# MSNLAB/Federated-Lifelong-Person-ReID

Hardware: AMD Instinct MI355X
Metric: images/sec (whole node) per fed round, fedstil resnet50 (higher is better)
Workload: dtype bf16; 1 GPU; model=resnet50-fedstil, global_batch=64, img=128x64, images_per_round_per_client=512, num_classes=8000, lambda_k=2000, rehearsal_set=2000 exemplar budget + task (m=32/id), parallelism=fed-dp1 (1 client/GPU)

## Files before the change

flreid_amd/models/resnet.py:

```python

from __future__ import annotations

from typing import List, Type, Union

import torch
import torch.nn as nn
import torch.nn.functional as F

from flreid_amd import ops
from flreid_amd.tools.logger import Logger
from flreid_amd.tools.winit import weights_init_classifier, weights_init_kaiming

_log = Logger("models.resnet")


class EvalFusedBatchNorm2d(nn.BatchNorm2d):

    fuse_relu = False

    def forward(self, x):
        if not self.training:
            out = ops.bn_eval_2d(x, self, relu=self.fuse_relu)
            if out is not None:
                return out
        else:
            out = ops.bn_train_2d(x, self, relu=self.fuse_relu)
            if out is not None:
                return out
        out = super().forward(x)
        return F.relu(out, inplace=True) if self.fuse_relu else out


class EvalFusedBatchNorm1d(nn.BatchNorm1d):

    def forward(self, x):
        if not self.training:
            out = ops.bn_eval_2d(x, self)
            if out is not None:
                return out
        else:
            out = ops.bn_train_2d(x, self)
            if out is not None:
                return out
        return super().forward(x)


class FusedConv3x3(nn.Conv2d):

    def forward(self, x):
        if self.stride == (1, 1) and self.bias is None:
            y = ops.conv3x3_try(x, self.weight)
            if y is not None:
                return y
        return super().forward(x)


def conv3x3(cin: int, cout: int, stride: int = 1) -> nn.Conv2d:
    return FusedConv3x3(cin, cout, 3, stride=stride, padding=1, bias=False)


def conv1x1(cin: int, cout: int, stride: int = 1) -> nn.Conv2d:
    return nn.Conv2d(cin, cout, 1, stride=stride, bias=False)


class BasicBlock(nn.Module):
    expansion = 1

    def __init__(self, cin: int, planes: int, stride: int = 1,
                 downsample: nn.Module = None):
        super().__init__()
        self.conv1 = conv3x3(cin, planes, stride)
        self.bn1 = EvalFusedBatchNorm2d(planes)
        self.bn1.fuse_relu = True
        self.relu = nn.ReLU(inplace=True)
        self.conv2 = conv3x3(planes, planes)
        self.bn2 = EvalFusedBatchNorm2d(planes)
        self.downsample = downsample

    def forward(self, x: torch.Tensor) -> torch.Tensor:
        identity = x if self.downsample is None else self.downsample(x)
        out = self.bn1(self.conv1(x))
        out = self.bn2(self.conv2(out))
        return self.relu(out + identity)


class Bottleneck(nn.Module):
    expansion = 4

    def __init__(self, cin: int, planes: int, stride: int = 1,
                 downsample: nn.Module = None):
        super().__init__()
        self.conv1 = conv1x1(cin, planes)
        self.bn1 = EvalFusedBatchNorm2d(planes)
        self.bn1.fuse_relu = True
        self.conv2 = conv3x3(planes, planes, stride)
        self.bn2 = EvalFusedBatchNorm2d(planes)
        self.bn2.fuse_relu = True
        self.conv3 = conv1x1(planes, planes * self.expansion)
        self.bn3 = EvalFusedBatchNorm2d(planes * self.expansion)
        self.relu = nn.ReLU(inplace=True)
        self.downsample = downsample

    def forward(self, x: torch.Tensor) -> torch.Tensor:
        identity = x if self.downsample is None else self.downsample(x)
        out = self.bn1(self.conv1(x))
        out = self.bn2(self.conv2(out))
        out = self.bn3(self.conv3(out))
        return self.relu(out + identity)


class ResNetTrunk(nn.Module):

    def __init__(self, block: Type[Union[BasicBlock, Bottleneck]],
                 layers: List[int], last_stride: int = 2):
        super().__init__()
        self.inplanes = 64
        self.conv1 = nn.Conv2d(3, 64, 7, stride=2, padding=3, bias=False)
        self.bn1 = EvalFusedBatchNorm2d(64)
        self.bn1.fuse_relu = True
        self.relu = nn.ReLU(inplace=True)
        self.maxpool = nn.MaxPool2d(3, stride=2, padding=1)
        self.layer1 = self._make_stage(block, 64, layers[0])
        self.layer2 = self._make_stage(block, 128, layers[1], stride=2)
        self.layer3 = self._make_stage(block, 256, layers[2], stride=2)
        self.layer4 = self._make_stage(block, 512, layers[3], stride=last_stride)
        self.avgpool = nn.AdaptiveAvgPool2d(1)
        self._init_weights()

    def _make_stage(self, block, planes: int, depth: int, stride: int = 1) -> nn.Sequential:
        downsample = None
        if stride != 1 or self.inplanes != planes * block.expansion:
            downsample = nn.Sequential(
                conv1x1(self.inplanes, planes * block.expansion, stride),
                EvalFusedBatchNorm2d(planes * block.expansion),
            )
        blocks = [block(self.inplanes, planes, stride, downsample)]
        self.inplanes = planes * block.expansion
        blocks += [block(self.inplanes, planes) for _ in range(1, depth)]
        return nn.Sequential(*blocks)

    def _init_weights(self) -> None:
        for m in self.modules():
            if isinstance(m, nn.Conv2d):
                nn.init.kaiming_normal_(m.weight, mode="fan_out", nonlinearity="relu")
            elif isinstance(m, nn.BatchNorm2d):
                nn.init.constant_(m.weight, 1.0)
                nn.init.constant_(m.bias, 0.0)

    def forward(self, x: torch.Tensor) -> torch.Tensor:
        x = self.maxpool(self.bn1(self.conv1(x)))
        x = self.layer4(self.layer3(self.layer2(self.layer1(x))))
        x = self.avgpool(x)
        return torch.flatten(x, 1)


_ARCH = {
    "resnet18": (BasicBlock, [2, 2, 2, 2], 512),
    "resnet34": (BasicBlock, [3, 4, 6, 3], 512),
    "resnet50": (Bottleneck, [3, 4, 6, 3], 2048),
    "resnet101": (Bottleneck, [3, 4, 23, 3], 2048),
    "resnet152": (Bottleneck, [3, 8, 36, 3], 2048),
}


class ResNetReID(nn.Module):
    def __init__(self, model_name: str, num_classes: int = 1000,
                 last_stride: int = 2, neck: str = "no",
                 pretrained: bool = False, **kwargs):
        super().__init__()
        for n, p in kwargs.items():
            setattr(self, n, p)
        if model_name not in _ARCH:
            raise ValueError(f"No model named {model_name}.")
        block, layers, self.in_planes = _ARCH[model_name]
        self.model_name = model_name
        self.num_classes = num_classes
        self.neck = neck
        self.base = ResNetTrunk(block, layers, last_stride=last_stride)

        if neck == "no":
            self.classifier = nn.Linear(self.in_planes, num_classes)
        elif neck == "bnneck":
            self.bottleneck = EvalFusedBatchNorm1d(self.in_planes)
            self.bottleneck.bias.requires_grad_(False)
            self.classifier = nn.Linear(self.in_planes, num_classes, bias=False)
            self.bottleneck.apply(weights_init_kaiming)
            self.classifier.apply(weights_init_classifier)
        else:
            raise ValueError(f"Mismatched neck type {neck}.")

# ... 58 lines not shown
```

flreid_amd/ops/__init__.py:

```python

from __future__ import annotations

import os
from collections import OrderedDict
from typing import Dict, Optional, Sequence, Tuple

import torch

from flreid_amd.ops import reference as ref

_EXT = None
_EXT_ERR: Optional[str] = None

_F32, _BF16 = 0, 1


def _load_extension():
    global _EXT, _EXT_ERR
    if _EXT is not None or _EXT_ERR is not None:
        return _EXT
    try:
        from flreid_amd.ops import _flreid_hip

        _EXT = _flreid_hip
# ... 770 lines not shown

def _penalty_meta(rows, n_sets: int, total: int, chunk: int):
    ptr_rows = [(p.data_ptr(), *(0 if t is None else t.data_ptr()
                                 for t in slots)) for p, slots in rows]
    key = (n_sets, rows[0][0].device,
           tuple((p.numel(), *pr) for (p, _), pr in zip(rows, ptr_rows)))
    meta = _PENALTY_META.get(key)
    if meta is not None:
        _PENALTY_META.move_to_end(key)
        return meta
    chunk_rows, offsets, flat_off = _chunk_table(
        [p.numel() for p, _ in rows], chunk, pad_to=4)
    assert flat_off == total
    dev = rows[0][0].device
    meta = (torch.tensor(ptr_rows, dtype=torch.int64, device=dev),
            torch.tensor(chunk_rows, dtype=torch.int32, device=dev),
            n_sets, offsets, total)
    _PENALTY_META[key] = meta
    while len(_PENALTY_META) > _PENALTY_META_CAP:
        _PENALTY_META.popitem(last=False)
    return meta


class _QuadraticPenaltyHipFn(torch.autograd.Function):

    @staticmethod
    def forward(ctx, meta, consts, *params):
        ext = _ext_or_raise("penalty_fwd")
        ptrs, chunks, n_sets, offsets, total = meta
        partials = torch.empty(chunks.shape[0], device=params[0].device,
                               dtype=torch.float32)
        ext.penalty_fwd(ptrs.data_ptr(), chunks.data_ptr(), n_sets,
                        partials.data_ptr(), chunks.shape[0], _stream())
        ctx.save_for_backward(*params)
        ctx.meta = meta
        ctx.consts = consts
        return partials.sum()

    @staticmethod
    def backward(ctx, grad_out):
        ext = _ext_or_raise("penalty_bwd")
        params = ctx.saved_tensors
        ptrs, chunks, n_sets, offsets, total = ctx.meta
        g = grad_out.to(torch.float32).contiguous()
        flat = torch.empty(total, device=g.device, dtype=torch.float32)
        ext.penalty_bwd(ptrs.data_ptr(), chunks.data_ptr(), n_sets,
                        g.data_ptr(), flat.data_ptr(), chunks.shape[0],
                        _stream())
        views = [torch.as_strided(flat, p.shape, p.stride(), off)
                 for p, off in zip(params, offsets)]
        return (None, None, *views)


def quadratic_penalty_sets(
        params: Dict[str, torch.Tensor],
        sets: Sequence[Tuple[Dict[str, torch.Tensor],
                             Optional[Dict[str, torch.Tensor]]]],
) -> torch.Tensor:
    sets = list(sets)
    first = next(iter(params.values()), None)
    if (sets and first is not None and first.is_cuda
            and os.environ.get("FLREID_NO_FUSED_PENALTY", "0") != "1"):
        plan = _penalty_plan(params, sets)
        if plan is not None:
            ext = _ext_or_raise("penalty_fwd")
            if ext is not None:
                rows, total = plan
                meta = _penalty_meta(rows, len(sets), total,
                                     ext.penalty_chunk())
                consts = tuple(t for _, slots in rows for t in slots
                               if t is not None)
                return _QuadraticPenaltyHipFn.apply(
                    meta, consts, *(p for p, _ in rows))
    return ref.quadratic_penalty_sets(params, sets)


def quadratic_penalty(params: Dict[str, torch.Tensor],
                      anchors: Dict[str, torch.Tensor],
                      importance: Optional[Dict[str, torch.Tensor]] = None,
                      ) -> torch.Tensor:
    return quadratic_penalty_sets(params, [(anchors, importance)])


class _BnTrain2dFn(torch.autograd.Function):

    @staticmethod
    def forward(ctx, x, gamma, beta, running_mean, running_var, momentum, eps,
                nbt, relu):
        ext = _ext_or_raise("bn_train")
        c = x.shape[1]
        m = x.numel() // c
        y = torch.empty_like(x)
        smean = torch.empty(c, device=x.device, dtype=torch.float32)
        sinv = torch.empty(c, device=x.device, dtype=torch.float32)
        nslab = ext.bn_train_nslab(m, c)
        part = torch.empty(2, nslab, c, device=x.device, dtype=torch.float32)
        has_rs = running_mean is not None
        ext.bn_train_fwd(
            x.data_ptr(), y.data_ptr(),
            gamma.detach().contiguous().data_ptr(),
            beta.detach().contiguous().data_ptr(),
            running_mean.data_ptr() if has_rs else 0,
            running_var.data_ptr() if has_rs else 0,
            smean.data_ptr(), sinv.data_ptr(),
            part[0].data_ptr(), part[1].data_ptr(),
            nbt.data_ptr() if nbt is not None else 0, m, c,
            float(momentum), float(eps), float(m) / float(m - 1),
            int(relu), _dt(x), _stream())
        ctx.save_for_backward(x, gamma, beta, smean, sinv)
        ctx.relu = bool(relu)
        return y

    @staticmethod
    def backward(ctx, dy):
        x, gamma, beta, smean, sinv = ctx.saved_tensors
        if x.dim() == 4:
            if not dy.is_contiguous(memory_format=torch.channels_last):
                dy = dy.contiguous(memory_format=torch.channels_last)
        elif not dy.is_contiguous():
            dy = dy.contiguous()
        if dy.dtype != x.dtype:
            dy = dy.to(x.dtype)
        ext = _ext_or_raise("bn_train")
        c = x.shape[1]
        m = x.numel() // c
        dx = torch.empty_like(x)
        dgamma = torch.empty(c, device=x.device, dtype=torch.float32)
        dbeta = torch.empty(c, device=x.device, dtype=torch.float32)
        nslab = ext.bn_train_nslab(m, c)
        part = torch.empty(2, nslab, c, device=x.device, dtype=torch.float32)
        ext.bn_train_bwd(x.data_ptr(), dy.data_ptr(), dx.data_ptr(),
                         gamma.detach().contiguous().data_ptr(),
                         beta.detach().contiguous().data_ptr(),
                         smean.data_ptr(), sinv.data_ptr(),
                         dgamma.data_ptr(), dbeta.data_ptr(),
                         part[0].data_ptr(), part[1].data_ptr(),
                         m, c, int(ctx.relu), _dt(x), _stream())
        return dx, dgamma, dbeta, None, None, None, None, None, None


def bn_train_2d(x: torch.Tensor, bn,
                relu: bool = False) -> Optional[torch.Tensor]:
    if os.environ.get("FLREID_NO_FUSED_BN", "0") == "1":
        return None
    if (not x.is_cuda or x.dtype not in (torch.float32, torch.bfloat16)
            or bn.weight is None or bn.bias is None):
        return None
    if x.dim() == 4:
        if not x.is_contiguous(memory_format=torch.channels_last):
            return None
    elif x.dim() == 2:
        if not x.is_contiguous():
            return None
    else:
        return None
    c = x.shape[1]
    m = x.numel() // c
    if c % 64 != 0 or m < 2 or m > 16384:
        return None
    if bn.momentum is None:
        return None
    if not extension_available():
        return None
    nbt = None
    if bn.track_running_stats and bn.running_mean is not None:
        nbt = bn.num_batches_tracked
        rm, rv = bn.running_mean, bn.running_var
    else:
        rm = rv = None
    return _BnTrain2dFn.apply(x, bn.weight, bn.bias, rm, rv,
                              bn.momentum, bn.eps, nbt, relu)


def _cl(t: torch.Tensor) -> torch.Tensor:
    return t if t.is_contiguous(memory_format=torch.channels_last) \
        else t.contiguous(memory_format=torch.channels_last)


def compose_theta_bf16(ext, gw: torch.Tensor, atten: Optional[torch.Tensor],
                       aw: Optional[torch.Tensor],
                       out: Optional[torch.Tensor] = None) -> torch.Tensor:
    gw_d = gw.detach()
    L, inner = atten_geometry(gw_d)
    if atten is not None and atten.numel() != L:
        if gw_d.dim() == 4 or not atten.numel() or L % atten.numel():
            raise ValueError(f"compose_theta_bf16: {atten.numel()} atten "
                             f"entries do not fit a last weight dim of {L}")
        L = atten.numel()
    if out is None:
        out = torch.empty_like(gw_d, dtype=torch.bfloat16)
    elif out.dtype != torch.bfloat16 or not same_layout(out, gw_d):
        raise ValueError("compose_theta_bf16: out must be bf16 in gw's layout")
    ext.compose2(gw_d.data_ptr(),
                 atten.detach().float().contiguous().data_ptr() if atten is not None else 0,
                 aw.detach().data_ptr() if aw is not None else 0,
                 out.data_ptr(), gw_d.numel(), L, inner, _dt(gw_d), _BF16,
                 _stream())
    return out


class _AdaptiveLinear1x1Fn(torch.autograd.Function):

    @staticmethod
    def forward(ctx, x, gw2d, atten, aw2d, bias):
        ext = _ext_or_raise("compose2")
        x_bf = x.detach().to(torch.bfloat16).contiguous()
        theta = compose_theta_bf16(ext, gw2d, atten, aw2d)
        y = x_bf @ theta.t()
        if bias is not None:
            y = y + bias.detach().to(torch.bfloat16)
        ctx.save_for_backward(x_bf, theta)
        ctx.x_dtype = x.dtype
        ctx.has_bias = bias is not None
        return y

    @staticmethod
    def backward(ctx, grad_out):
        x_bf, theta = ctx.saved_tensors
        g = grad_out.to(torch.bfloat16)
        dx = (g @ theta).to(ctx.x_dtype)
        d_aw = (g.t() @ x_bf).to(torch.float32)
        d_bias = grad_out.sum(0).to(torch.float32) if ctx.has_bias else None
        return dx, None, None, d_aw, d_bias


class _ThetaLinearFn(torch.autograd.Function):

    @staticmethod
    def forward(ctx, x, theta, bias, k2):
        x_bf = x.detach().to(torch.bfloat16).contiguous()
        th = theta.detach()
        if k2:
            ext = _ext_or_raise("theta_linear_fwd")
            m, k = x_bf.shape
            n = th.shape[0]
            y = torch.empty(m, n, device=x.device, dtype=torch.bfloat16)
            ext.theta_linear_fwd(
                x_bf.data_ptr(), th.data_ptr(),
                bias.detach().contiguous().float().data_ptr()
                if bias is not None else 0,
                y.data_ptr(), m, n, k, _stream())
        else:
            y = x_bf @ th.t()
            if bias is not None:
                y = y + bias.detach().to(torch.bfloat16)
        ctx.save_for_backward(x_bf, th)
        ctx.x_dtype = x.dtype
        ctx.has_bias = bias is not None
        return y

    @staticmethod
    def backward(ctx, grad_out):
        x_bf, th = ctx.saved_tensors
        g = grad_out.to(torch.bfloat16)
# ... 311 lines not shown
```

flreid_amd/ops/csrc/bn_train.hip:

```cpp

#include "common.h"
#include "ops.h"

namespace flreid {

template <typename T>
__device__ __forceinline__ void bn_load4(const T* p, float v[4]);

template <>
__device__ __forceinline__ void bn_load4<float>(const float* p, float v[4]) {
  const float4 t = *reinterpret_cast<const float4*>(p);
  v[0] = t.x; v[1] = t.y; v[2] = t.z; v[3] = t.w;
}

template <>
__device__ __forceinline__ void bn_load4<__hip_bfloat16>(
    const __hip_bfloat16* p, float v[4]) {
  const ushort4 t = *reinterpret_cast<const ushort4*>(p);
  v[0] = __bfloat162float(*(const __hip_bfloat16*)&t.x);
  v[1] = __bfloat162float(*(const __hip_bfloat16*)&t.y);
  v[2] = __bfloat162float(*(const __hip_bfloat16*)&t.z);
  v[3] = __bfloat162float(*(const __hip_bfloat16*)&t.w);
}

template <typename T>
__device__ __forceinline__ void bn_store4(T* p, const float v[4]);

template <>
__device__ __forceinline__ void bn_store4<float>(float* p, const float v[4]) {
  *reinterpret_cast<float4*>(p) = float4{v[0], v[1], v[2], v[3]};
}

template <>
__device__ __forceinline__ void bn_store4<__hip_bfloat16>(
    __hip_bfloat16* p, const float v[4]) {
  ushort4 t;
  __hip_bfloat16 b;
  b = __float2bfloat16(v[0]); t.x = *(const unsigned short*)&b;
  b = __float2bfloat16(v[1]); t.y = *(const unsigned short*)&b;
  b = __float2bfloat16(v[2]); t.z = *(const unsigned short*)&b;
  b = __float2bfloat16(v[3]); t.w = *(const unsigned short*)&b;
  *reinterpret_cast<ushort4*>(p) = t;
}

constexpr int BN_STRIPES = 16;
constexpr int BN_CG = 64;

template <typename T, bool IS_BWD>
__global__ __launch_bounds__(256) void bn_partial_kernel(
    const T* __restrict__ X, const T* __restrict__ DY,
    const float* __restrict__ smean, const float* __restrict__ sinv,
    const float* __restrict__ gamma, const float* __restrict__ beta,
    float* __restrict__ part_a, float* __restrict__ part_b, int64_t M,
    int C, int relu) {
  const int c0 = blockIdx.x * BN_CG;
  const int q = threadIdx.x & 15;
  const int r = threadIdx.x >> 4;
  const int c = c0 + q * 4;
  const int S = gridDim.y * BN_STRIPES;
  const int g = blockIdx.y * BN_STRIPES + r;

  __shared__ float la[BN_STRIPES][BN_CG + 4];
  __shared__ float lb[BN_STRIPES][BN_CG + 4];

  float mn[4], iv[4], sc[4], sh[4];
  if (IS_BWD) {
#pragma unroll
    for (int j = 0; j < 4; ++j) {
      mn[j] = smean[c + j];
      iv[j] = sinv[c + j];
      if (relu) {
        sc[j] = gamma[c + j] * iv[j];
        sh[j] = beta[c + j] - mn[j] * sc[j];
      }
    }
  }

  float sa[4] = {0.f, 0.f, 0.f, 0.f};
  float sb[4] = {0.f, 0.f, 0.f, 0.f};
  for (int64_t row = g; row < M; row += S) {
    float x[4];
    bn_load4(X + row * C + c, x);
// ... 152 lines not shown
      float d = dy[j];
      if (relu && x[j] * g_iv[j] + sh[j] <= 0.f) d = 0.f;
      dx[j] = g_iv[j] * (d - mdy[j] - xhat * mdyx[j]);
    }
    bn_store4(DX + row * C + c, dx);
  }
}

static int bn_nslab(int64_t M, int C) {
  const int cg = C / BN_CG;
  int ns = 256 / cg;
  const int max_rows = (int)((M + BN_STRIPES - 1) / BN_STRIPES);
  if (ns > max_rows) ns = max_rows;
  if (ns > 64) ns = 64;
  if (ns < 1) ns = 1;
  return ns;
}

extern "C" int flreid_bn_train_nslab(int64_t M, int C) {
  return bn_nslab(M, C);
}

extern "C" void flreid_bn_train_fwd(const void* X, void* Y, const float* gamma,
                                    const float* beta, float* rmean,
                                    float* rvar, float* smean, float* sinv,
                                    float* part_a, float* part_b,
                                    unsigned long long* nbt, int64_t M, int C,
                                    float momentum, float eps, float unbiased,
                                    int relu, int dtype, hipStream_t stream) {
  if (C % BN_CG != 0) throw std::runtime_error("bn_train: C % 64 != 0");
  dim3 grid(C / BN_CG, bn_nslab(M, C)), block(256);
  if (dtype == kBF16) {
    hipLaunchKernelGGL((bn_partial_kernel<__hip_bfloat16, false>), grid,
                       block, 0, stream, (const __hip_bfloat16*)X, nullptr,
                       nullptr, nullptr, nullptr, nullptr, part_a, part_b, M,
                       C, 0);
    hipLaunchKernelGGL(bn_finalize_fwd_kernel<__hip_bfloat16>, grid, block, 0,
                       stream, (const __hip_bfloat16*)X, (__hip_bfloat16*)Y,
                       gamma, beta, rmean, rvar, smean, sinv, part_a, part_b,
                       nbt, M, C, momentum, eps, unbiased, relu);
  } else {
    hipLaunchKernelGGL((bn_partial_kernel<float, false>), grid, block, 0,
                       stream, (const float*)X, nullptr, nullptr, nullptr,
                       nullptr, nullptr, part_a, part_b, M, C, 0);
    hipLaunchKernelGGL(bn_finalize_fwd_kernel<float>, grid, block, 0, stream,
                       (const float*)X, (float*)Y, gamma, beta, rmean, rvar,
                       smean, sinv, part_a, part_b, nbt, M, C, momentum, eps,
                       unbiased, relu);
  }
  HIP_CHECK(hipGetLastError());
}

extern "C" void flreid_bn_train_bwd(const void* X, const void* DY, void* DX,
                                    const float* gamma, const float* beta,
                                    const float* smean, const float* sinv,
                                    float* dgamma, float* dbeta,
                                    float* part_a, float* part_b, int64_t M,
                                    int C, int relu, int dtype,
                                    hipStream_t stream) {
  if (C % BN_CG != 0) throw std::runtime_error("bn_train: C % 64 != 0");
  dim3 grid(C / BN_CG, bn_nslab(M, C)), block(256);
  if (dtype == kBF16) {
    hipLaunchKernelGGL((bn_partial_kernel<__hip_bfloat16, true>), grid, block,
                       0, stream, (const __hip_bfloat16*)X,
                       (const __hip_bfloat16*)DY, smean, sinv, gamma, beta,
                       part_a, part_b, M, C, relu);
    hipLaunchKernelGGL(bn_finalize_bwd_kernel<__hip_bfloat16>, grid, block, 0,
                       stream, (const __hip_bfloat16*)X,
                       (const __hip_bfloat16*)DY, (__hip_bfloat16*)DX, gamma,
                       beta, smean, sinv, dgamma, dbeta, part_a, part_b, M, C,
                       relu);
  } else {
    hipLaunchKernelGGL((bn_partial_kernel<float, true>), grid, block, 0,
                       stream, (const float*)X, (const float*)DY, smean, sinv,
                       gamma, beta, part_a, part_b, M, C, relu);
    hipLaunchKernelGGL(bn_finalize_bwd_kernel<float>, grid, block, 0, stream,
                       (const float*)X, (const float*)DY, (float*)DX, gamma,
                       beta, smean, sinv, dgamma, dbeta, part_a, part_b, M, C,
                       relu);
  }
  HIP_CHECK(hipGetLastError());
}

}
```

flreid_amd/ops/csrc/module.cpp:

```cpp

#include <pybind11/pybind11.h>
#include <pybind11/stl.h>

#include <cstdint>
#include <stdexcept>
#include <string>
#include <vector>

#include "ops.h"

namespace py = pybind11;
using namespace flreid;

template <typename T> struct py_arg {
  using type = T;
  static T to(T v) { return v; }
};
template <typename T> struct py_arg<T*> {
  using type = uintptr_t;
  static T* to(uintptr_t v) { return reinterpret_cast<T*>(v); }
};
template <auto Fn> struct binder;
template <typename R, typename... A, R (*Fn)(A...)> struct binder<Fn> {
  static R call(typename py_arg<A>::type... a) {
    return Fn(py_arg<A>::to(a)...);
  }
};

#define FLREID_DEF(name) m.def(#name, &binder<&flreid_##name>::call)

PYBIND11_MODULE(_flreid_hip, m) {
  m.doc() = "flreid MI355X (gfx950) kernels";

  FLREID_DEF(l2norm_rows);
  FLREID_DEF(ce_smooth);
  FLREID_DEF(compose);
  FLREID_DEF(compose2);
  FLREID_DEF(bn_eval);
  FLREID_DEF(pairwise);
  FLREID_DEF(rowsq);
  FLREID_DEF(window_attn_fwd);
  FLREID_DEF(window_attn_bwd);
  FLREID_DEF(triplet_fwd);
  FLREID_DEF(triplet_bwd);
  FLREID_DEF(adaptive_linear_fwd);
  FLREID_DEF(theta_linear_fwd);
  FLREID_DEF(conv3x3_fwd);
  FLREID_DEF(conv3x3_tile);
  FLREID_DEF(conv3x3_img_fwd);
  FLREID_DEF(conv3x3_img_fwd_ldsw);
  FLREID_DEF(conv3x3_wgrad);
  FLREID_DEF(transpose_bf16);
  FLREID_DEF(bn_train_nslab);
  FLREID_DEF(bn_train_fwd);
  FLREID_DEF(bn_train_bwd);
  FLREID_DEF(drift_fwd);
  FLREID_DEF(drift_bwd);
  FLREID_DEF(kd_fwd);
  FLREID_DEF(icarl_distill);
  FLREID_DEF(patch_merge_ln_fwd);
  FLREID_DEF(patch_merge_ln_bwd);
  FLREID_DEF(decomposed_fwd);
  FLREID_DEF(decomposed_bwd);
  FLREID_DEF(head_step_chunk);
  FLREID_DEF(penalty_chunk);
  FLREID_DEF(penalty_block);
  FLREID_DEF(penalty_fwd);
  FLREID_DEF(penalty_bwd);


  m.def("importance",
        [](uintptr_t F, uintptr_t g, int64_t numel, int dtype, bool sq,
           float scale, uintptr_t stream) {
          flreid_importance((float*)F, (const void*)g, numel, dtype,
                            sq ? 1 : 0, scale, (hipStream_t)stream);
        });

  m.def("decomposed_plan",
        [](int64_t rows, int64_t C, int64_t S, int channels_last) {
          int64_t tpr = 0, blocks = 0;
          flreid_decomposed_plan(rows, C, S, channels_last, &tpr, &blocks);
          return py::make_tuple(tpr, blocks);
        });

  m.def("head_step",
        [](const std::vector<std::vector<int64_t>>& rows, uintptr_t partials,
           int64_t n_partials, double lr, double beta1, double beta2,
           double weight_decay, double eps, float lambda, uintptr_t stream) {
          std::vector<int64_t> flat;
          flat.reserve(rows.size() * kHeadStepFields);
          for (const auto& r : rows) {
            if (r.size() != kHeadStepFields)
              throw std::invalid_argument(
                  "head_step: rows need " + std::to_string(kHeadStepFields) +
                  " fields");
            flat.insert(flat.end(), r.begin(), r.end());
          }
          flreid_head_step(flat.data(), (int)rows.size(), (double*)partials,
                           n_partials, lr, beta1, beta2, weight_decay, eps,
                           lambda, (hipStream_t)stream);
        });
}
```

flreid_amd/ops/csrc/ops.h:

```cpp
#pragma once

#include <hip/hip_runtime.h>

#include <cstdint>

namespace flreid {

constexpr int kHeadStepFields = 14;

extern "C" {

void flreid_l2norm_rows(const void* x, void* y, int64_t rows, int64_t cols,
                        int dtype, float eps, hipStream_t stream);
void flreid_ce_smooth(const void* score, const int64_t* target,
                      float* row_loss, void* grad, int64_t B, int64_t C,
                      int dtype, float eps, hipStream_t stream);
void flreid_compose(const void* gw, const float* atten, const void* aw,
                    void* out, int64_t numel, int64_t L, int dtype,
                    hipStream_t stream);
void flreid_compose2(const void* gw, const float* atten, const void* aw,
                     void* out, int64_t numel, int64_t L, int64_t inner,
                     int in_dtype, int out_dtype, hipStream_t stream);
void flreid_importance(float* F, const void* g, int64_t numel, int dtype,
                       int sq, float scale, hipStream_t stream);
void flreid_bn_eval(const void* x, void* y, const float* gamma,
                    const float* beta, const float* mean, const float* var,
                    int64_t numel, int C, int64_t HW, float eps, int nhwc,
                    int relu, int dtype, hipStream_t stream);

void flreid_pairwise(const float* A, const float* B, const float* aa,
                     const float* bb, float* out, int64_t M, int64_t N,
                     int64_t D, int mode, hipStream_t stream);
void flreid_rowsq(const float* x, float* out, int64_t rows, int64_t cols,
                  hipStream_t stream);

void flreid_window_attn_fwd(const void* q, const void* k, const void* v,
                            const float* bias, const float* mask, void* out,
                            int64_t BW, int H, int N, int D, int nW,
                            float scale, int dtype, hipStream_t stream);
void flreid_window_attn_bwd(const void* q, const void* k, const void* v,
                            const float* bias, const float* mask,
                            const void* dout, void* dq, void* dk, void* dv,
                            float* ds, int64_t BW, int H, int N, int D, int nW,
                            float scale, int dtype, hipStream_t stream);

void flreid_triplet_fwd(const float* F, const float* norms,
                        const int64_t* labels, float* row_loss, int* p_idx,
                        int* n_idx, int N, int D, float margin,
                        hipStream_t stream);
void flreid_triplet_bwd(const float* F, const float* row_loss,
                        const int* p_idx, const int* n_idx, float* grad, int N,
                        int D, float coeff, hipStream_t stream);

void flreid_adaptive_linear_fwd(const void* X, const float* GW,
                                const float* AW, const float* ATTEN,
                                const float* BIAS, void* OUT, int M, int N,
                                int K, int split_layout, hipStream_t stream);
void flreid_theta_linear_fwd(const void* x, const void* theta,
                             const float* bias, void* out, int M, int N, int K,
                             hipStream_t stream);

void flreid_conv3x3_fwd(const void* x, const float* w, void* y, int NB, int H,
                        int Wd, int C, int K, hipStream_t stream);

void flreid_conv3x3_tile(const void* gw, const float* atten, const void* aw,
                         void* out, int C, int K, int in_dtype, int mode,
                         hipStream_t stream);
void flreid_conv3x3_img_fwd(const void* x, const void* w, void* y, int NB,
                            int H, int Wd, int C, int K, hipStream_t stream);
void flreid_transpose_bf16(const void* in, void* out, int64_t M, int64_t N,
                           hipStream_t stream);
void flreid_conv3x3_wgrad(const void* dy, const void* x, float* dw, int NB,
                          int H, int Wd, int C, int K, hipStream_t stream);

void flreid_conv3x3_img_fwd_ldsw(const void* x, const void* w, void* y, int NB,
                                 int H, int Wd, int C, int K,
                                 hipStream_t stream);

int flreid_bn_train_nslab(int64_t M, int C);
void flreid_bn_train_fwd(const void* x, void* y, const float* gamma,
                         const float* beta, float* rmean, float* rvar,
                         float* smean, float* sinv, float* part_a,
                         float* part_b, unsigned long long* nbt, int64_t M,
                         int C, float momentum, float eps, float unbiased,
                         int relu, int dtype, hipStream_t stream);
void flreid_bn_train_bwd(const void* x, const void* dy, void* dx,
                         const float* gamma, const float* beta,
                         const float* smean, const float* sinv, float* dgamma,
                         float* dbeta, float* part_a, float* part_b, int64_t M,
                         int C, int relu, int dtype, hipStream_t stream);

void flreid_drift_fwd(const int64_t* ptrs, const int* chunks, float* partials,
                      int n_chunks, hipStream_t stream);
void flreid_drift_bwd(const int64_t* ptrs, const int* chunks,
                      const float* gscale, float* flat_grad, int n_chunks,
                      hipStream_t stream);

void flreid_kd_fwd(const float* zs, const float* zt, float* row_loss,
                   float* grad, int64_t B, int64_t C, float temperature,
                   hipStream_t stream);
void flreid_icarl_distill(const float* score, const int64_t* target,
                          const float* prev, float* row_loss, float* grad,
                          int64_t B, int64_t C, int64_t P, hipStream_t stream);

void flreid_patch_merge_ln_fwd(const void* x, const float* gamma,
                               const float* beta, void* y, float* mean,
                               float* rstd, int64_t rows, int C, int H, int W,
                               float eps, int dtype, hipStream_t stream);
void flreid_patch_merge_ln_bwd(const void* x, const float* gamma,
                               const void* dy, const float* mean,
                               const float* rstd, void* dx, float* dg,
                               float* db, int64_t rows, int C, int H, int W,
                               int dtype, hipStream_t stream);

void flreid_decomposed_plan(int64_t rows, int64_t C, int64_t S,
                            int channels_last, int64_t* tasks_per_row,
                            int64_t* blocks);
void flreid_decomposed_fwd(const float* sw, const float* mask, const float* aw,
                           const float* aw_kb, const float* atten, void* out,
                           int64_t rows, int64_t C, int64_t S, int64_t KB,
                           int channels_last, int train, float lambda_l1,
                           float lambda_mask, int out_dtype,
                           hipStream_t stream);
void flreid_decomposed_bwd(const void* g, int g_dtype, const float* sw,
                           const float* mask, const float* aw,
                           const float* aw_kb, float* d_aw, float* dmask_part,
                           float* datten_part, int64_t rows, int64_t C,
                           int64_t S, int64_t KB, int channels_last, int train,
                           float lambda_l1, float lambda_mask, int need_aw,
                           int need_mask, int need_atten, hipStream_t stream);

int flreid_head_step_chunk();
void flreid_head_step(const int64_t* rows, int n_rows, double* partials,
                      int64_t n_partials, double lr, double beta1,
                      double beta2, double weight_decay, double eps,
                      float lambda, hipStream_t stream);

int flreid_penalty_chunk();
int flreid_penalty_block();
void flreid_penalty_fwd(const int64_t* ptrs, const int* chunks, int S,
                        float* partials, int n_chunks, hipStream_t stream);
void flreid_penalty_bwd(const int64_t* ptrs, const int* chunks, int S,
                        const float* gscale, float* flat_grad, int n_chunks,
                        hipStream_t stream);

}

}
```

Measured before the change: 5260 images/sec.

## Add single-launch training BatchNorm kernels with fused residual add and ReLU

```diff
diff --git a/flreid_amd/models/resnet.py b/flreid_amd/models/resnet.py
--- a/flreid_amd/models/resnet.py
+++ b/flreid_amd/models/resnet.py
@@ -1,7 +1,8 @@
 
 from __future__ import annotations
 
-from typing import List, Type, Union
+import os
+from typing import List, Optional, Type, Union
 
 import torch
 import torch.nn as nn
@@ -29,6 +30,12 @@
                 return out
         out = super().forward(x)
         return F.relu(out, inplace=True) if self.fuse_relu else out
+
+    def forward_add_relu(self, x, identity) -> Optional[torch.Tensor]:
+        if (not self.training or self.fuse_relu or not x.is_cuda
+                or os.environ.get("FLREID_BN_RESIDUAL", "1") == "0"):
+            return None
+        return ops.bn_train_2d(x, self, residual=identity)
 
 
 class EvalFusedBatchNorm1d(nn.BatchNorm1d):
@@ -80,7 +87,11 @@
     def forward(self, x: torch.Tensor) -> torch.Tensor:
         identity = x if self.downsample is None else self.downsample(x)
         out = self.bn1(self.conv1(x))
-        out = self.bn2(self.conv2(out))
+        out = self.conv2(out)
+        fused = self.bn2.forward_add_relu(out, identity)
+        if fused is not None:
+            return fused
+        out = self.bn2(out)
         return self.relu(out + identity)
 
 
@@ -105,7 +116,11 @@
         identity = x if self.downsample is None else self.downsample(x)
         out = self.bn1(self.conv1(x))
         out = self.bn2(self.conv2(out))
-        out = self.bn3(self.conv3(out))
+        out = self.conv3(out)
+        fused = self.bn3.forward_add_relu(out, identity)
+        if fused is not None:
+            return fused
+        out = self.bn3(out)
         return self.relu(out + identity)
 
 
diff --git a/flreid_amd/ops/__init__.py b/flreid_amd/ops/__init__.py
--- a/flreid_amd/ops/__init__.py
+++ b/flreid_amd/ops/__init__.py
@@ -876,38 +876,67 @@
     return quadratic_penalty_sets(params, [(anchors, importance)])
 
 
+def _bn_onepass(ext, m: int, c: int, dt: int) -> bool:
+    if os.environ.get("FLREID_BN_TRAIN_IMPL", "auto") == "split":
+        return False
+    return bool(ext.bn_train_onepass_ok(m, c, dt))
+
+
 class _BnTrain2dFn(torch.autograd.Function):
 
     @staticmethod
     def forward(ctx, x, gamma, beta, running_mean, running_var, momentum, eps,
-                nbt, relu):
+                nbt, relu, residual):
         ext = _ext_or_raise("bn_train")
         c = x.shape[1]
         m = x.numel() // c
         y = torch.empty_like(x)
         smean = torch.empty(c, device=x.device, dtype=torch.float32)
         sinv = torch.empty(c, device=x.device, dtype=torch.float32)
-        nslab = ext.bn_train_nslab(m, c)
-        part = torch.empty(2, nslab, c, device=x.device, dtype=torch.float32)
         has_rs = running_mean is not None
-        ext.bn_train_fwd(
-            x.data_ptr(), y.data_ptr(),
-            gamma.detach().contiguous().data_ptr(),
-            beta.detach().contiguous().data_ptr(),
-            running_mean.data_ptr() if has_rs else 0,
-            running_var.data_ptr() if has_rs else 0,
-            smean.data_ptr(), sinv.data_ptr(),
-            part[0].data_ptr(), part[1].data_ptr(),
-            nbt.data_ptr() if nbt is not None else 0, m, c,
-            float(momentum), float(eps), float(m) / float(m - 1),
-            int(relu), _dt(x), _stream())
-        ctx.save_for_backward(x, gamma, beta, smean, sinv)
+        onepass = _bn_onepass(ext, m, c, _dt(x))
+        if residual is not None and not onepass:
+            raise RuntimeError("bn_train: residual needs the one-launch path")
+        if onepass:
+            ext.bn_train_fwd_onepass(
+                x.data_ptr(),
+                residual.data_ptr() if residual is not None else 0,
+                y.data_ptr(),
+                gamma.detach().contiguous().data_ptr(),
+                beta.detach().contiguous().data_ptr(),
+                running_mean.data_ptr() if has_rs else 0,
+                running_var.data_ptr() if has_rs else 0,
+                smean.data_ptr(), sinv.data_ptr(),
+                nbt.data_ptr() if nbt is not None else 0, m, c,
+                float(momentum), float(eps), float(m) / float(m - 1),
+                int(relu), 0, _dt(x), _stream())
+        else:
+            nslab = ext.bn_train_nslab(m, c)
+            part = torch.empty(2, nslab, c, device=x.device,
+                               dtype=torch.float32)
+            ext.bn_train_fwd(
+                x.data_ptr(), y.data_ptr(),
+                gamma.detach().contiguous().data_ptr(),
+                beta.detach().contiguous().data_ptr(),
+                running_mean.data_ptr() if has_rs else 0,
+                running_var.data_ptr() if has_rs else 0,
+                smean.data_ptr(), sinv.data_ptr(),
+                part[0].data_ptr(), part[1].data_ptr(),
+                nbt.data_ptr() if nbt is not None else 0, m, c,
+                float(momentum), float(eps), float(m) / float(m - 1),
+                int(relu), _dt(x), _stream())
+        if residual is not None:
+            ctx.save_for_backward(x, gamma, beta, smean, sinv, y)
+        else:
+            ctx.save_for_backward(x, gamma, beta, smean, sinv)
         ctx.relu = bool(relu)
+        ctx.onepass = onepass
+        ctx.has_residual = residual is not None
         return y
 
     @staticmethod
     def backward(ctx, dy):
-        x, gamma, beta, smean, sinv = ctx.saved_tensors
+        x, gamma, beta, smean, sinv = ctx.saved_tensors[:5]
         if x.dim() == 4:
             if not dy.is_contiguous(memory_format=torch.channels_last):
                 dy = dy.contiguous(memory_format=torch.channels_last)
@@ -921,20 +950,38 @@
         dx = torch.empty_like(x)
         dgamma = torch.empty(c, device=x.device, dtype=torch.float32)
         dbeta = torch.empty(c, device=x.device, dtype=torch.float32)
-        nslab = ext.bn_train_nslab(m, c)
-        part = torch.empty(2, nslab, c, device=x.device, dtype=torch.float32)
-        ext.bn_train_bwd(x.data_ptr(), dy.data_ptr(), dx.data_ptr(),
-                         gamma.detach().contiguous().data_ptr(),
-                         beta.detach().contiguous().data_ptr(),
-                         smean.data_ptr(), sinv.data_ptr(),
-                         dgamma.data_ptr(), dbeta.data_ptr(),
-                         part[0].data_ptr(), part[1].data_ptr(),
-                         m, c, int(ctx.relu), _dt(x), _stream())
-        return dx, dgamma, dbeta, None, None, None, None, None, None
-
-
-def bn_train_2d(x: torch.Tensor, bn,
-                relu: bool = False) -> Optional[torch.Tensor]:
+        d_res = None
+        if ctx.onepass:
+            y = ctx.saved_tensors[5] if ctx.has_residual else None
+            if y is not None:
+                d_res = torch.empty_like(x)
+            ext.bn_train_bwd_onepass(
+                x.data_ptr(), dy.data_ptr(),
+                y.data_ptr() if y is not None else 0, dx.data_ptr(),
+                d_res.data_ptr() if d_res is not None else 0,
+                gamma.detach().contiguous().data_ptr(),
+                beta.detach().contiguous().data_ptr(),
+                smean.data_ptr(), sinv.data_ptr(),
+                dgamma.data_ptr(), dbeta.data_ptr(),
+                m, c, int(ctx.relu), 0, _dt(x), _stream())
+        else:
+            nslab = ext.bn_train_nslab(m, c)
+            part = torch.empty(2, nslab, c, device=x.device,
+                               dtype=torch.float32)
+            ext.bn_train_bwd(x.data_ptr(), dy.data_ptr(), dx.data_ptr(),
+                             gamma.detach().contiguous().data_ptr(),
+                             beta.detach().contiguous().data_ptr(),
+                             smean.data_ptr(), sinv.data_ptr(),
+                             dgamma.data_ptr(), dbeta.data_ptr(),
+                             part[0].data_ptr(), part[1].data_ptr(),
+                             m, c, int(ctx.relu), _dt(x), _stream())
+        return (dx, dgamma, dbeta, None, None, None, None, None, None,
+                d_res)
+
+
+def bn_train_2d(x: torch.Tensor, bn, relu: bool = False,
+                residual: Optional[torch.Tensor] = None,
+                ) -> Optional[torch.Tensor]:
     if os.environ.get("FLREID_NO_FUSED_BN", "0") == "1":
         return None
     if (not x.is_cuda or x.dtype not in (torch.float32, torch.bfloat16)
@@ -956,6 +1003,12 @@
         return None
     if not extension_available():
         return None
+    if residual is not None:
+        if (not residual.is_cuda or residual.dtype != x.dtype
+                or residual.shape != x.shape
+                or residual.stride() != x.stride()
+                or not _bn_onepass(_ext_or_raise("bn_train"), m, c, _dt(x))):
+            return None
     nbt = None
     if bn.track_running_stats and bn.running_mean is not None:
         nbt = bn.num_batches_tracked
@@ -963,7 +1016,7 @@
     else:
         rm = rv = None
     return _BnTrain2dFn.apply(x, bn.weight, bn.bias, rm, rv,
-                              bn.momentum, bn.eps, nbt, relu)
+                              bn.momentum, bn.eps, nbt, relu, residual)
 
 
 def _cl(t: torch.Tensor) -> torch.Tensor:
diff --git a/flreid_amd/ops/csrc/bn_train.hip b/flreid_amd/ops/csrc/bn_train.hip
--- a/flreid_amd/ops/csrc/bn_train.hip
+++ b/flreid_amd/ops/csrc/bn_train.hip
@@ -1,3 +1,5 @@
+
+#include <type_traits>
 
 #include "common.h"
 #include "ops.h"
@@ -316,4 +318,509 @@
   HIP_CHECK(hipGetLastError());
 }
 
-}
+#pragma clang fp contract(off)
+
+constexpr int BN1_THREADS = 256;
+constexpr int BN1_XBYTES = 128;
+constexpr int BN1_LDS_MAX = 64 * 1024;
+
+template <int NW>
+struct alignas(NW * 4) bn_pk {
+  uint32_t w[NW];
+};
+
+template <typename T, int CB, int VEC>
+struct bn1_geom {
+  static constexpr int L = CB / VEC;
+  static constexpr int SLOTS = BN1_THREADS / L;
+  static constexpr int NW = VEC * (int)sizeof(T) / 4;
+  static constexpr int NR = BN1_XBYTES / (VEC * (int)sizeof(T));
+  using pk = bn_pk<NW>;
+};
+
+template <typename T, int VEC>
+__device__ __forceinline__ void bn1_unpack(
+    const bn_pk<VEC * (int)sizeof(T) / 4>& p, float v[VEC]) {
+  if constexpr (sizeof(T) == 4) {
+#pragma unroll
+    for (int j = 0; j < VEC; ++j) v[j] = __uint_as_float(p.w[j]);
+  } else {
+#pragma unroll
+    for (int j = 0; j < VEC / 2; ++j) {
+      v[2 * j] = __uint_as_float(p.w[j] << 16);
+      v[2 * j + 1] = __uint_as_float(p.w[j] & 0xffff0000u);
+    }
+  }
+}
+
+__device__ __forceinline__ uint32_t bn1_bf16_bits(float v) {
+  const __hip_bfloat16 b = __float2bfloat16(v);
+  return *(const unsigned short*)&b;
+}
+
+template <typename T, int VEC>
+__device__ __forceinline__ void bn1_pack(
+    const float v[VEC], bn_pk<VEC * (int)sizeof(T) / 4>& p) {
+  if constexpr (sizeof(T) == 4) {
+#pragma unroll
+    for (int j = 0; j < VEC; ++j) p.w[j] = __float_as_uint(v[j]);
+  } else {
+#pragma unroll
+    for (int j = 0; j < VEC / 2; ++j)
+      p.w[j] = bn1_bf16_bits(v[2 * j]) | (bn1_bf16_bits(v[2 * j + 1]) << 16);
+  }
+}
+
+template <typename T>
+__device__ __forceinline__ float bn1_round(float v) {
+  if constexpr (sizeof(T) == 4) {
+    return v;
+  } else {
+    return __uint_as_float(bn1_bf16_bits(v) << 16);
+  }
+}
+
+__device__ __forceinline__ int bn1_group(int b, int nb) {
+  return (nb % 8 == 0) ? (b % 8) * (nb / 8) + b / 8 : b;
+}
+
+__host__ __device__ constexpr int bn1_slab_stride(int cb) {
+  return (BN_STRIPES + 1) * cb;
+}
+static size_t bn1_lds_bytes(int nslab, int cb) {
+  return sizeof(float) *
+         (2 * (size_t)nslab * bn1_slab_stride(cb) + 2 * (size_t)nslab * cb +
+          2 * cb);
+}
+
+template <int CB>
+__device__ __forceinline__ void bn1_reduce(const float* la, const float* lb,
+                                           float* sla, float* slb, int nslab,
+                                           float& ta, float& tb) {
+  __syncthreads();
+  for (int t = threadIdx.x; t < nslab * CB; t += BN1_THREADS) {
+    const int s = t / CB, ch = t % CB;
+    const float* pa = la + s * bn1_slab_stride(CB) + ch;
+    const float* pb = lb + s * bn1_slab_stride(CB) + ch;
+    float xa = 0.f, xb = 0.f;
+#pragma unroll
+    for (int i = 0; i < BN_STRIPES; ++i) {
+      xa += pa[i * CB];
+      xb += pb[i * CB];
+    }
+    sla[t] = xa;
+    slb[t] = xb;
+  }
+  __syncthreads();
+  ta = 0.f;
+  tb = 0.f;
+  if (threadIdx.x < CB) {
+    for (int s = 0; s < nslab; ++s) {
+      ta += sla[s * CB + threadIdx.x];
+      tb += slb[s * CB + threadIdx.x];
+    }
+  }
+}
+
+#define BN1_ROWS_BEGIN                                                       \
+  {                                                                          \
+    int g = slot, i = 0;                                                     \
+    _Pragma("unroll") for (int k = 0; k < G::NR; ++k) {                      \
+      if (k < nit) {                                                         \
+        const int row = g + i * S;                                           \
+        const bool valid = (g < S) & (row < Mi);                             \
+        const uint32_t boff = (uint32_t)row * rowb + colb;                   \
+        const bool last = i + 1 == nrs;
+#define BN1_ROWS_END                                                         \
+        if (last) { i = 0; g += G::SLOTS; } else { ++i; }                    \
+      }                                                                      \
+    }                                                                        \
+  }
+
+template <typename P>
+__device__ __forceinline__ P bn1_ld(const void* base, uint32_t boff) {
+  return *reinterpret_cast<const P*>((const char*)base + boff);
+}
+template <typename P>
+__device__ __forceinline__ void bn1_st(void* base, uint32_t boff, const P& v) {
+  *reinterpret_cast<P*>((char*)base + boff) = v;
+}
+
+template <typename T, int CB, int VEC>
+__global__ __launch_bounds__(BN1_THREADS) void bn_onepass_fwd_kernel(
+    const T* __restrict__ X, const T* __restrict__ R, T* __restrict__ Y,
+    const float* __restrict__ gamma, const float* __restrict__ beta,
+    float* __restrict__ rmean, float* __restrict__ rvar,
+    float* __restrict__ smean, float* __restrict__ sinv,
+    unsigned long long* __restrict__ nbt, int64_t M, int C, int nslab,
+    float momentum, float eps, float unbiased, int relu) {
+  using G = bn1_geom<T, CB, VEC>;
+  using pk = typename G::pk;
+  extern __shared__ float bn1_lds[];
+  float* la = bn1_lds;
+  float* lb = la + nslab * bn1_slab_stride(CB);
+  float* sla = lb + nslab * bn1_slab_stride(CB);
+  float* slb = sla + nslab * CB;
+  float* lmean = slb + nslab * CB;
+  float* linv = lmean + CB;
+
+  const int Mi = (int)M;
+  const int S = nslab * BN_STRIPES;
+  const int nrs = (Mi + S - 1) / S;
+  const int nit = ((S + G::SLOTS - 1) / G::SLOTS) * nrs;
+  const int slot = threadIdx.x / G::L;
+  const int cl = (threadIdx.x % G::L) * VEC;
+  const int c0 = bn1_group(blockIdx.x, gridDim.x) * CB;
+  const int col = c0 + cl;
+  const uint32_t rowb = (uint32_t)C * sizeof(T);
+  const uint32_t colb = (uint32_t)col * sizeof(T);
+
+  if (nbt != nullptr && blockIdx.x == 0 && threadIdx.x == 0) ++(*nbt);
+
+  pk xr[G::NR];
+#pragma unroll
+  for (int k = 0; k < G::NR; ++k) xr[k] = pk{};
+  BN1_ROWS_BEGIN { if (valid) xr[k] = bn1_ld<pk>(X, boff); } BN1_ROWS_END
+
+  {
+    float sa[VEC], sb[VEC];
+#pragma unroll
+    for (int j = 0; j < VEC; ++j) sa[j] = sb[j] = 0.f;
+    BN1_ROWS_BEGIN {
+      float x[VEC];
+      bn1_unpack<T, VEC>(xr[k], x);
+#pragma unroll
+      for (int j = 0; j < VEC; ++j) {
+        sa[j] += x[j];
+        sb[j] = __builtin_fmaf(x[j], x[j], sb[j]);
+      }
+      if (last) {
+        if (g < S) {
+          const int o = (g / BN_STRIPES) * bn1_slab_stride(CB) +
+                        (g % BN_STRIPES) * CB + cl;
+#pragma unroll
+          for (int j = 0; j < VEC; ++j) {
+            la[o + j] = sa[j];
+            lb[o + j] = sb[j];
+          }
+        }
+#pragma unroll
+        for (int j = 0; j < VEC; ++j) sa[j] = sb[j] = 0.f;
+      }
+    } BN1_ROWS_END
+  }
+
+  float ta, tb;
+  bn1_reduce<CB>(la, lb, sla, slb, nslab, ta, tb);
+  if (threadIdx.x < CB) {
+    const float inv_m = 1.f / (float)M;
+    const float mean = ta * inv_m;
+    const float var = fmaxf(__builtin_fmaf(-mean, mean, tb * inv_m), 0.f);
+    const float inv = rsqrtf(var + eps);
+    lmean[threadIdx.x] = mean;
+    linv[threadIdx.x] = inv;
+    const int gc = c0 + threadIdx.x;
+    smean[gc] = mean;
+    sinv[gc] = inv;
+    if (rmean != nullptr) {
+      rmean[gc] = (1.f - momentum) * rmean[gc] + momentum * mean;
+      rvar[gc] = (1.f - momentum) * rvar[gc] + momentum * var * unbiased;
+    }
+  }
+  __syncthreads();
+
+  float scale[VEC], shift[VEC];
+#pragma unroll
+  for (int j = 0; j < VEC; ++j) {
+    scale[j] = gamma[col + j] * linv[cl + j];
+    shift[j] = __builtin_fmaf(-scale[j], lmean[cl + j], beta[col + j]);
+  }
+  if (R != nullptr) {
+    BN1_ROWS_BEGIN {
+      if (valid) {
+        const pk rp = bn1_ld<pk>(R, boff);
+        float v[VEC], r[VEC];
+        bn1_unpack<T, VEC>(xr[k], v);
+        bn1_unpack<T, VEC>(rp, r);
+#pragma unroll
+        for (int j = 0; j < VEC; ++j) {
+          const float b =
+              bn1_round<T>(__builtin_fmaf(v[j], scale[j], shift[j]));
+          v[j] = fmaxf(b + r[j], 0.f);
+        }
+        pk out;
+        bn1_pack<T, VEC>(v, out);
+        bn1_st<pk>(Y, boff, out);
+      }
+    } BN1_ROWS_END
+  } else {
+    BN1_ROWS_BEGIN {
+      if (valid) {
+        float v[VEC];
+        bn1_unpack<T, VEC>(xr[k], v);
+#pragma unroll
+        for (int j = 0; j < VEC; ++j) {
+          v[j] = __builtin_fmaf(v[j], scale[j], shift[j]);
+          if (relu) v[j] = fmaxf(v[j], 0.f);
+        }
+        pk out;
+        bn1_pack<T, VEC>(v, out);
+        bn1_st<pk>(Y, boff, out);
+      }
+    } BN1_ROWS_END
+  }
+}
+
+template <typename T, int CB, int VEC>
+__global__ __launch_bounds__(BN1_THREADS) void bn_onepass_bwd_kernel(
+    const T* __restrict__ X, const T* __restrict__ DY,
+    const T* __restrict__ YS, T* __restrict__ DX, T* __restrict__ DR,
+    const float* __restrict__ gamma, const float* __restrict__ beta,
+    const float* __restrict__ smean, const float* __restrict__ sinv,
+    float* __restrict__ dgamma, float* __restrict__ dbeta, int64_t M, int C,
+    int nslab, int relu) {
+  using G = bn1_geom<T, CB, VEC>;
+  using pk = typename G::pk;
+  extern __shared__ float bn1_lds[];
+  float* la = bn1_lds;
+  float* lb = la + nslab * bn1_slab_stride(CB);
+  float* sla = lb + nslab * bn1_slab_stride(CB);
+  float* slb = sla + nslab * CB;
+  float* lmdy = slb + nslab * CB;
+  float* lmdyx = lmdy + CB;
+
+  const int Mi = (int)M;
+  const int S = nslab * BN_STRIPES;
+  const int nrs = (Mi + S - 1) / S;
+  const int nit = ((S + G::SLOTS - 1) / G::SLOTS) * nrs;
+  const int slot = threadIdx.x / G::L;
+  const int cl = (threadIdx.x % G::L) * VEC;
+  const int c0 = bn1_group(blockIdx.x, gridDim.x) * CB;
+  const int col = c0 + cl;
+  const uint32_t rowb = (uint32_t)C * sizeof(T);
+  const uint32_t colb = (uint32_t)col * sizeof(T);
+  const bool mask_sign = relu && YS == nullptr;
+
+  pk xr[G::NR], dr[G::NR];
+#pragma unroll
+  for (int k = 0; k < G::NR; ++k) xr[k] = dr[k] = pk{};
+  BN1_ROWS_BEGIN {
+    if (valid) {
+      xr[k] = bn1_ld<pk>(X, boff);
+      dr[k] = bn1_ld<pk>(DY, boff);
+    }
+  } BN1_ROWS_END
+  if (YS != nullptr) {
+    BN1_ROWS_BEGIN {
+      if (valid) {
+        const pk yp = bn1_ld<pk>(YS, boff);
+        float y[VEC], d[VEC];
+        bn1_unpack<T, VEC>(yp, y);
+        bn1_unpack<T, VEC>(dr[k], d);
+#pragma unroll
+        for (int j = 0; j < VEC; ++j)
+          if (y[j] <= 0.f) d[j] = 0.f;
+        bn1_pack<T, VEC>(d, dr[k]);
+        bn1_st<pk>(DR, boff, dr[k]);
+      }
+    } BN1_ROWS_END
+  }
+
+  float mn[VEC], iv[VEC], g_iv[VEC], sh[VEC];
+#pragma unroll
+  for (int j = 0; j < VEC; ++j) {
+    mn[j] = smean[col + j];
+    iv[j] = sinv[col + j];
+    g_iv[j] = gamma[col + j] * iv[j];
+    sh[j] = 0.f;
+    if (mask_sign) sh[j] = __builtin_fmaf(-mn[j], g_iv[j], beta[col + j]);
+  }
+  {
+    float sa[VEC], sb[VEC];
+#pragma unroll
+    for (int j = 0; j < VEC; ++j) sa[j] = sb[j] = 0.f;
+    BN1_ROWS_BEGIN {
+      float x[VEC], dy[VEC];
+      bn1_unpack<T, VEC>(xr[k], x);
+      bn1_unpack<T, VEC>(dr[k], dy);
+#pragma unroll
+      for (int j = 0; j < VEC; ++j) {
+        if (mask_sign && __builtin_fmaf(x[j], g_iv[j], sh[j]) <= 0.f)
+          continue;
+        sa[j] += dy[j];
+        sb[j] = __builtin_fmaf(dy[j] * (x[j] - mn[j]), iv[j], sb[j]);
+      }
+      if (last) {
+        if (g < S) {
+          const int o = (g / BN_STRIPES) * bn1_slab_stride(CB) +
+                        (g % BN_STRIPES) * CB + cl;
+#pragma unroll
+          for (int j = 0; j < VEC; ++j) {
+            la[o + j] = sa[j];
+            lb[o + j] = sb[j];
+          }
+        }
+#pragma unroll
+        for (int j = 0; j < VEC; ++j) sa[j] = sb[j] = 0.f;
+      }
+    } BN1_ROWS_END
+  }
+
+  float tdy, tdyx;
+  bn1_reduce<CB>(la, lb, sla, slb, nslab, tdy, tdyx);
+  if (threadIdx.x < CB) {
+    const int gc = c0 + threadIdx.x;
+    dgamma[gc] = tdyx;
+    dbeta[gc] = tdy;
+    const float inv_m = 1.f / (float)M;
+    lmdy[threadIdx.x] = tdy * inv_m;
+    lmdyx[threadIdx.x] = tdyx * inv_m;
+  }
+  __syncthreads();
+
+  float mdy[VEC], mdyx[VEC];
+#pragma unroll
+  for (int j = 0; j < VEC; ++j) {
+    mdy[j] = lmdy[cl + j];
+    mdyx[j] = lmdyx[cl + j];
+  }
+  BN1_ROWS_BEGIN {
+    if (valid) {
+      float x[VEC], dy[VEC], dx[VEC];
+      bn1_unpack<T, VEC>(xr[k], x);
+      bn1_unpack<T, VEC>(dr[k], dy);
+#pragma unroll
+      for (int j = 0; j < VEC; ++j) {
+        const float xhat = (x[j] - mn[j]) * iv[j];
+        float d = dy[j];
+        if (mask_sign && __builtin_fmaf(x[j], g_iv[j], sh[j]) <= 0.f) d = 0.f;
+        dx[j] = g_iv[j] * __builtin_fmaf(-xhat, mdyx[j], d - mdy[j]);
+      }
+      pk out;
+      bn1_pack<T, VEC>(dx, out);
+      bn1_st<pk>(DX, boff, out);
+    }
+  } BN1_ROWS_END
+}
+#undef BN1_ROWS_BEGIN
+#undef BN1_ROWS_END
+
+static int bn1_vec(int64_t M, int C, int es, int cb) {
+  if (C <= 0 || C % BN_CG != 0 || C > 16384 || M < 2 || M > 16384) return 0;
+  if (cb != 4 && cb != 8 && cb != 16) return 0;
+  const int nslab = bn_nslab(M, C);
+  if (bn1_lds_bytes(nslab, cb) > (size_t)BN1_LDS_MAX) return 0;
+  const int S = nslab * BN_STRIPES;
+  const int nrs = (int)((M + S - 1) / S);
+  for (int vb = 16; vb >= 8; vb /= 2) {
+    const int vec = vb / es;
+    if (vec > cb) continue;
+    const int slots = BN1_THREADS / (cb / vec);
+    const int spt = (S + slots - 1) / slots;
+    if (spt * nrs <= BN1_XBYTES / vb) return vec;
+  }
+  return 0;
+}
+
+static int bn1_auto_cb(int64_t M, int C, int dtype) {
+  const int es = dtype == kBF16 ? 2 : 4;
+  const int first = C >= 1024 ? 8 : 4;
+  if (bn1_vec(M, C, es, first) != 0) return first;
+  if (bn1_vec(M, C, es, 12 - first) != 0) return 12 - first;
+  return 0;
+}
+
+extern "C" int flreid_bn_train_onepass_ok(int64_t M, int C, int dtype) {
+  if (dtype != kBF16 && dtype != kF32) return 0;
+  return bn1_auto_cb(M, C, dtype) != 0 ? 1 : 0;
+}
+
+template <int V>
+using bn1_int = std::integral_constant<int, V>;
+template <typename T>
+struct bn1_type { using type = T; };
+
+template <typename T, typename F>
+static void bn1_dispatch(int cb, int vec, F&& f) {
+  constexpr int V16 = 16 / (int)sizeof(T), V8 = 8 / (int)sizeof(T);
+  bool hit = false;
+  auto one = [&](auto cbc, auto vc) {
+    if (!hit && cb == decltype(cbc)::value && vec == decltype(vc)::value) {
+      hit = true;
+      f(cbc, vc);
+    }
+  };
+  if constexpr (V16 <= 4) one(bn1_int<4>{}, bn1_int<V16>{});
+  one(bn1_int<4>{}, bn1_int<V8>{});
+  one(bn1_int<8>{}, bn1_int<V16>{});
+  one(bn1_int<8>{}, bn1_int<V8>{});
+  one(bn1_int<16>{}, bn1_int<V16>{});
+  one(bn1_int<16>{}, bn1_int<V8>{});
+  if (!hit) throw std::runtime_error("bn_train onepass: no kernel for cb/vec");
+}
+
+static void bn1_plan(int64_t M, int C, int dtype, int& cb, int& vec) {
+  if (dtype != kBF16 && dtype != kF32)
+    throw std::runtime_error("bn_train onepass: dtype");
+  if (cb == 0) cb = bn1_auto_cb(M, C, dtype);
+  vec = bn1_vec(M, C, dtype == kBF16 ? 2 : 4, cb);
+  if (vec == 0)
+    throw std::runtime_error(
+        "bn_train onepass: shape not eligible (see flreid_bn_train_onepass_ok)");
+}
+
+extern "C" void flreid_bn_train_fwd_onepass(
+    const void* X, const void* residual, void* Y, const float* gamma,
+    const float* beta, float* rmean, float* rvar, float* smean, float* sinv,
+    unsigned long long* nbt, int64_t M, int C, float momentum, float eps,
+    float unbiased, int relu, int cb, int dtype, hipStream_t stream) {
+  int vec = 0;
+  bn1_plan(M, C, dtype, cb, vec);
+  const int nslab = bn_nslab(M, C);
+  const dim3 grid(C / cb), block(BN1_THREADS);
+  const size_t lds = bn1_lds_bytes(nslab, cb);
+  auto go = [&](auto tag) {
+    using T = typename decltype(tag)::type;
+    bn1_dispatch<T>(cb, vec, [&](auto cbc, auto vc) {
+      hipLaunchKernelGGL(
+          (bn_onepass_fwd_kernel<T, decltype(cbc)::value,
+                                 decltype(vc)::value>),
+          grid, block, lds, stream, (const T*)X, (const T*)residual, (T*)Y,
+          gamma, beta, rmean, rvar, smean, sinv, nbt, M, C, nslab, momentum,
+          eps, unbiased, relu);
+    });
+  };
+  if (dtype == kBF16) go(bn1_type<__hip_bfloat16>{});
+  else go(bn1_type<float>{});
+  HIP_CHECK(hipGetLastError());
+}
+
+extern "C" void flreid_bn_train_bwd_onepass(
+    const void* X, const void* DY, const void* y_saved, void* DX,
+    void* d_residual, const float* gamma, const float* beta,
+    const float* smean, const float* sinv, float* dgamma, float* dbeta,
+    int64_t M, int C, int relu, int cb, int dtype, hipStream_t stream) {
+  if ((y_saved == nullptr) != (d_residual == nullptr))
+    throw std::runtime_error("bn_train onepass: y_saved without d_residual");
+  int vec = 0;
+  bn1_plan(M, C, dtype, cb, vec);
+  const int nslab = bn_nslab(M, C);
+  const dim3 grid(C / cb), block(BN1_THREADS);
+  const size_t lds = bn1_lds_bytes(nslab, cb);
+  auto go = [&](auto tag) {
+    using T = typename decltype(tag)::type;
+    bn1_dispatch<T>(cb, vec, [&](auto cbc, auto vc) {
+      hipLaunchKernelGGL(
+          (bn_onepass_bwd_kernel<T, decltype(cbc)::value,
+                                 decltype(vc)::value>),
+          grid, block, lds, stream, (const T*)X, (const T*)DY,
+          (const T*)y_saved, (T*)DX, (T*)d_residual, gamma, beta, smean, sinv,
+          dgamma, dbeta, M, C, nslab, relu);
+    });
+  };
+  if (dtype == kBF16) go(bn1_type<__hip_bfloat16>{});
+  else go(bn1_type<float>{});
+  HIP_CHECK(hipGetLastError());
+}
+
+}
diff --git a/flreid_amd/ops/csrc/module.cpp b/flreid_amd/ops/csrc/module.cpp
--- a/flreid_amd/ops/csrc/module.cpp
+++ b/flreid_amd/ops/csrc/module.cpp
@@ -54,6 +54,9 @@
   FLREID_DEF(bn_train_nslab);
   FLREID_DEF(bn_train_fwd);
   FLREID_DEF(bn_train_bwd);
+  FLREID_DEF(bn_train_onepass_ok);
+  FLREID_DEF(bn_train_fwd_onepass);
+  FLREID_DEF(bn_train_bwd_onepass);
   FLREID_DEF(drift_fwd);
   FLREID_DEF(drift_bwd);
   FLREID_DEF(kd_fwd);
diff --git a/flreid_amd/ops/csrc/ops.h b/flreid_amd/ops/csrc/ops.h
--- a/flreid_amd/ops/csrc/ops.h
+++ b/flreid_amd/ops/csrc/ops.h
@@ -89,6 +89,21 @@
                          const float* smean, const float* sinv, float* dgamma,
                          float* dbeta, float* part_a, float* part_b, int64_t M,
                          int C, int relu, int dtype, hipStream_t stream);
+int flreid_bn_train_onepass_ok(int64_t M, int C, int dtype);
+void flreid_bn_train_fwd_onepass(const void* x, const void* residual, void* y,
+                                 const float* gamma, const float* beta,
+                                 float* rmean, float* rvar, float* smean,
+                                 float* sinv, unsigned long long* nbt,
+                                 int64_t M, int C, float momentum, float eps,
+                                 float unbiased, int relu, int cb, int dtype,
+                                 hipStream_t stream);
+void flreid_bn_train_bwd_onepass(const void* x, const void* dy,
+                                 const void* y_saved, void* dx,
+                                 void* d_residual, const float* gamma,
+                                 const float* beta, const float* smean,
+                                 const float* sinv, float* dgamma,
+                                 float* dbeta, int64_t M, int C, int relu,
+                                 int cb, int dtype, hipStream_t stream);
 
 void flreid_drift_fwd(const int64_t* ptrs, const int* chunks, float* partials,
                       int n_chunks, hipStream_t stream);
```

Result: no change. 5225 images/sec (-0.7%).
